# ZihaoW123/UniMM

Hardware: AMD Instinct MI355X
Metric: dialog-sequences/sec (fwd+bwd) at bs=240 seq=256 regions=36(+1 <IMG>) (higher is better)
Workload: dtype bf16; 1 GPU; UniMM-UL sparse training step (BASELINE configs[1]): bert_base_6layer_6conect, sequences_per_image=6, num_negative_samples=5, mask_prob=0.15, dropout on, MLM+UL / NSP / region-KL losses, fwd+bwd, optimizer step not included; global_batch=240, per_gpu_batch=240, seq_len=256, regions=37, parallelism=dp1, executor=eager launches, step_api=loss = combine(losses); loss.backward() (autograd, as train.py:164-168, :315)

## Files before the change

### unimm_amd/csrc/attention.hip

```cpp
#include <type_traits>
#include "common.h"

namespace {

struct AttnParams {
  const bf16_t* q; const bf16_t* k; const bf16_t* v;
  bf16_t* o; float* lse;
  const uint32_t* mask;
  const int* q_off; const int* q_len; const int* k_off; const int* k_len;
  const int* ks_off; const int* ks_len; int ks_ins;
  const int* order;
  int B, H, Tq, Tk, ldq, ldk, ldv, ldo;
  int mask_q_stride, mask_b_stride;
  int parts;
  float scale;
  DropoutArg drop;
};

constexpr float LOG2E = 1.4426950408889634f;
constexpr float LN2 = 0.6931471805599453f;

template <int D> __device__ __forceinline__ int swz(int row) {
  if constexpr (D == 64) { const int t = row >> 1; return (t & 7) ^ ((t & 1) << 2); }
  else return ((row & 3) << 2) | ((row >> 2) & 3);
}

template <int D>
__device__ __forceinline__ void stage_head(const bf16_t* __restrict__ g, int ld, int nrows, int nrows_pad,
                                           char* img, int tid, int nthreads) {
  constexpr int CPR = D / 8;
  constexpr int RPI = 64 / CPR;
  const int wave = tid >> 6, lane = tid & 63, nwaves = nthreads >> 6;
  const int rl = lane / CPR, pc = lane % CPR;
  for (int grp = wave; grp < nrows_pad / RPI; grp += nwaves) {
    const int row = grp * RPI + rl;
    if (row < nrows) {
      const bf16_t* src = g + (size_t)row * ld + ((pc ^ swz<D>(row)) << 3);
      __builtin_amdgcn_global_load_lds(GLB_PTR(src), LDS_PTR(img + grp * 1024), 16, 0, 0);
    } else {
      *reinterpret_cast<u32x4*>(img + grp * 1024 + lane * 16) = u32x4{0u, 0u, 0u, 0u};
    }
  }
}
template <int D>
__device__ __forceinline__ void stage_head_seg(const bf16_t* __restrict__ base, int ld, size_t kbase, size_t sbase, int ins, int slen,
                                               int nrows, int nrows_pad, char* img, int tid, int nthreads) {
  constexpr int CPR = D / 8, RPI = 64 / CPR;
  const int wave = tid >> 6, lane = tid & 63, nwaves = nthreads >> 6;
  const int rl = lane / CPR, pc = lane % CPR;
  for (int grp = wave; grp < nrows_pad / RPI; grp += nwaves) {
    const int row = grp * RPI + rl;
    if (row < nrows) {
      const size_t grow = row < ins ? kbase + row : (row < ins + slen ? sbase + (row - ins) : kbase + (row - slen));
      const bf16_t* src = base + grow * ld + ((pc ^ swz<D>(row)) << 3);
      __builtin_amdgcn_global_load_lds(GLB_PTR(src), LDS_PTR(img + grp * 1024), 16, 0, 0);
    } else {
      *reinterpret_cast<u32x4*>(img + grp * 1024 + lane * 16) = u32x4{0u, 0u, 0u, 0u};
    }
  }
}
__device__ __forceinline__ void stage_wait() { asm volatile("s_waitcnt vmcnt(0)" ::: "memory"); }

template <int D> __device__ __forceinline__ bf16x8 read_row_frag(const char* img, int row, int chunk) {
  return *reinterpret_cast<const bf16x8*>(img + row * (2 * D) + ((chunk ^ swz<D>(row)) << 4));
}

template <int D>
__device__ __forceinline__ bf16x8 read_tr_frag(const char* img, int rowbase, int col0, int lane) {
  const int h = lane >> 5, i = lane & 15, qq = i >> 2, pp = i & 3;
  const int col = col0 + 16 * ((lane >> 4) & 1) + 4 * pp;
  typedef __attribute__((ext_vector_type(8))) short s16x8;
  s16x4 part[2];
#pragma unroll
  for (int jj = 0; jj < 2; ++jj) {
    const int row = rowbase + 8 * jj + 4 * h + qq;
    const int pch = (col >> 3) ^ swz<D>(row);
    part[jj] = __builtin_amdgcn_ds_read_tr16_b64_v4i16(
        (__attribute__((address_space(3))) s16x4*)LDS_PTR(img + row * (2 * D) + pch * 16 + (col & 7) * 2));
  }
  s16x8 v = {part[0][0], part[0][1], part[0][2], part[0][3], part[1][0], part[1][1], part[1][2], part[1][3]};
  return __builtin_bit_cast(bf16x8, v);
}

__device__ __forceinline__ bf16x8 pack8(const float* p) {
  typedef __attribute__((ext_vector_type(4))) unsigned int u4;
  u4 w = {pack2bf(p[0], p[1]), pack2bf(p[2], p[3]), pack2bf(p[4], p[5]), pack2bf(p[6], p[7])};
  return __builtin_bit_cast(bf16x8, w);
}

__device__ __forceinline__ int key_of_reg(int reg, int h) { return (reg & 3) + 8 * (reg >> 2) + 4 * h; }

template <int D>
__device__ __forceinline__ void store_acc_row(bf16_t* __restrict__ g, const f32x16 (&a)[D / 32], float s, int h, bool ok) {
#pragma unroll
  for (int dt = 0; dt < D / 32; ++dt)
#pragma unroll
    for (int qp = 0; qp < 2; ++qp) {
      const uint32_t a0 = pack2bf(a[dt][8 * qp] * s, a[dt][8 * qp + 1] * s), a1 = pack2bf(a[dt][8 * qp + 2] * s, a[dt][8 * qp + 3] * s);
      const uint32_t b0 = pack2bf(a[dt][8 * qp + 4] * s, a[dt][8 * qp + 5] * s), b1 = pack2bf(a[dt][8 * qp + 6] * s, a[dt][8 * qp + 7] * s);
      const auto w0 = __builtin_amdgcn_permlane32_swap(a0, b0, false, false);
      const auto w1 = __builtin_amdgcn_permlane32_swap(a1, b1, false, false);
      if (ok) *reinterpret_cast<u32x4*>(g + 32 * dt + 16 * qp + 8 * h) = u32x4{w0[0], w1[0], w0[1], w1[1]};
    }
}

template <int D, int NKT>
__global__ __launch_bounds__(512, 2) void attn_fwd_kernel(AttnParams p) {
  drop_resolve(p.drop);
  extern __shared__ __attribute__((aligned(16))) char smem[];
  constexpr int KPAD = NKT * 32;
  char* kimg = smem;
  char* vimg = smem + KPAD * 2 * D;
  const int tid = threadIdx.x, wave = tid >> 6, lane = tid & 63;
  const int item = blockIdx.x / p.parts, part = blockIdx.x % p.parts;
  const int b = p.order != nullptr ? p.order[item / p.H] : item / p.H, head = item % p.H;
  const int nwv = blockDim.x >> 6;
  const int r = lane & 31, h = lane >> 5;

  const int Ts_b = p.ks_len ? p.ks_len[b] : 0;
  int Tk_b = (p.k_len ? p.k_len[b] : p.Tk) + Ts_b;
  Tk_b = Tk_b < KPAD ? Tk_b : KPAD;
  const int Tq_b = p.q_len ? p.q_len[b] : p.Tq;
  if (part * (int)(blockDim.x >> 6) * 32 >= Tq_b) return;
  const size_t qbase = p.q_off ? (size_t)p.q_off[b] : (size_t)b * p.Tq;
  const size_t kbase = p.k_off ? (size_t)p.k_off[b] : (size_t)b * p.Tk;
  const size_t sbase = p.ks_off ? (size_t)p.ks_off[b] : 0;
  const int kpad_b = ((Tk_b + 31) & ~31) < KPAD ? ((Tk_b + 31) & ~31) : KPAD;
  stage_head_seg<D>(p.k + head * D, p.ldk, kbase, sbase, p.ks_ins, Ts_b, Tk_b, kpad_b, kimg, tid, blockDim.x);
  stage_head_seg<D>(p.v + head * D, p.ldv, kbase, sbase, p.ks_ins, Ts_b, Tk_b, kpad_b, vimg, tid, blockDim.x);

  int wt = part * nwv + wave;
  int q0, qrow;
  bool qvalid;
  bf16x8 qf[D / 16];
  uint32_t mw[NKT];
#define UNIMM_LOAD_QTILE()                                                                                    \
  {                                                                                                          \
    q0 = wt * 32;                                                                                            \
    qrow = q0 + r;                                                                                           \
    qvalid = qrow < Tq_b;                                                                                    \
    if (!qvalid) qrow = Tq_b - 1;                                                                            \
    const bf16_t* qg_ = p.q + (qbase + qrow) * p.ldq + head * D;                                             \
    _Pragma("unroll") for (int ks = 0; ks < D / 16; ++ks) qf[ks] = *reinterpret_cast<const bf16x8*>(qg_ + 16 * ks + 8 * h); \
    const uint32_t* mp_ = p.mask + (size_t)b * p.mask_b_stride + (size_t)qrow * p.mask_q_stride;            \
    _Pragma("unroll") for (int t = 0; t < NKT; ++t) mw[t] = 32 * t < p.Tk ? mp_[t] : 0u;    \
  }
  UNIMM_LOAD_QTILE()
  stage_wait();
  __syncthreads();
  constexpr bool WALK = D == 64;
  for (bool first = true; wt * 32 < Tq_b && (WALK || first); first = false, wt += nwv * p.parts) {
    if (WALK && !first) UNIMM_LOAD_QTILE()

  f32x16 s[NKT];
#pragma unroll
  for (int t = 0; t < NKT; ++t) {
    f32x16 acc = {};
    if (32 * t < Tk_b) {
#pragma unroll
      for (int ks = 0; ks < D / 16; ++ks) {
        const bf16x8 kf = read_row_frag<D>(kimg, 32 * t + r, 2 * ks + h);
        acc = __builtin_amdgcn_mfma_f32_32x32x16_bf16(kf, qf[ks], acc, 0, 0, 0);
      }
    }
    s[t] = acc;
  }

  const float c1 = p.scale * LOG2E;
  constexpr float MOFF = -10000.0f * LOG2E;
  int tk_here = Tk_b;
  asm volatile("" : "+v"(tk_here));
  float mx = -INFINITY;
#pragma unroll
  for (int t = 0; t < NKT; ++t) {
    if (32 * t >= Tk_b) continue;
    const uint32_t wn = ~(mw[t] >> (4 * h));
    auto scores = [&](auto partial) {
#pragma unroll
      for (int e = 0; e < 16; e += 2) {
        const int kk = (e & 3) + 8 * (e >> 2);
        f32x2v madd;
#pragma unroll
        for (int u = 0; u < 2; ++u) {
          const uint32_t mb = (uint32_t)__builtin_amdgcn_sbfe((int)wn, kk + u, 1) & __builtin_bit_cast(uint32_t, MOFF);
          madd[u] = __uint_as_float(mb);
          if constexpr (decltype(partial)::value)
// ... 26 lines not shown
  if (p.drop.thr != 0u) {
    const uint32_t wl = drop_lin(p.drop, drop_wbase(((uint32_t)b * p.H + head) * p.Tq + (uint32_t)qrow, (uint32_t)p.Tk, 0u) + 2u * (uint32_t)h);
#pragma unroll
    for (int t = 0; t < NKT; ++t) {
      if (32 * t >= Tk_b) continue;
#pragma unroll
      for (int e = 0; e < 16; e += 2) {
        const uint32_t w = drop_fin(p.drop, wl + (uint32_t)((32 * t + key_of_reg(e, 0)) >> 1) * DROP_M1);
        s[t][e] = drop_keep(p.drop, w, 0u) ? s[t][e] : 0.0f;
        s[t][e + 1] = drop_keep(p.drop, w, 1u) ? s[t][e + 1] : 0.0f;
      }
    }
  }

  f32x16 o[D / 32];
#pragma unroll
  for (int dt = 0; dt < D / 32; ++dt) o[dt] = f32x16{};
#pragma unroll
  for (int t = 0; t < NKT; ++t) {
    if (32 * t >= Tk_b) continue;
#pragma unroll
    for (int ss = 0; ss < 2; ++ss) {
      float pv[8];
#pragma unroll
      for (int j = 0; j < 8; ++j) pv[j] = s[t][8 * ss + j];
      const bf16x8 pf = pack8(pv);
#pragma unroll
      for (int dt = 0; dt < D / 32; ++dt) {
        const bf16x8 vf = read_tr_frag<D>(vimg, 32 * t + 16 * ss, 32 * dt, lane);
        o[dt] = __builtin_amdgcn_mfma_f32_32x32x16_bf16(vf, pf, o[dt], 0, 0, 0);
      }
    }
  }

  store_acc_row<D>(p.o + (qbase + (qvalid ? qrow : 0)) * p.ldo + head * D, o, inv, h, qvalid);
  if (qvalid) {
    if (p.lse != nullptr && h == 0) p.lse[((size_t)b * p.H + head) * p.Tq + qrow] = (mx + __log2f(sum)) * LN2;
  }
  }
#undef UNIMM_LOAD_QTILE
}


struct AttnBwdParams {
  const bf16_t* q; const bf16_t* k; const bf16_t* v; const bf16_t* o; const bf16_t* dout;
  const float* lse; float* delta;
  bf16_t* dq; bf16_t* dk; bf16_t* dv;
  const uint32_t* mask;
  const int* q_off; const int* q_len; const int* k_off; const int* k_len;
  const int* order;
  int B, H, Tq, Tk, ldq, ldk, ldv, ldo, lddo, lddq, lddk, lddv;
  int mask_q_stride, mask_b_stride;
  int parts;
  float scale;
  DropoutArg drop;
};

template <int D, int NKT>
__global__ __launch_bounds__(512, 2) void attn_bwd_dq_kernel(AttnBwdParams p) {
  drop_resolve(p.drop);
  extern __shared__ __attribute__((aligned(16))) char smem[];
  constexpr int KPAD = NKT * 32;
  char* kimg = smem;
  char* vimg = smem + KPAD * 2 * D;
  const int tid = threadIdx.x, wave = tid >> 6, lane = tid & 63;
  const int item = blockIdx.x / p.parts, part = blockIdx.x % p.parts;
// ... 266 lines not shown

template <int D>
__device__ __forceinline__ void bwd_stage_row_stats(const AttnBwdParams& p, int b, int head, size_t qbase, int Tq_b, int Tk_b, int qpad_b,
                                                    float* lse_s, float* del_s, uint32_t* mw_s, int mstride, int tid, int nthreads) {
  constexpr int LPR = D / 8;
  for (int i = tid; i < qpad_b; i += nthreads) {
    const size_t stat = ((size_t)b * p.H + head) * p.Tq + i;
    lse_s[i] = i < Tq_b ? -p.lse[stat] * LOG2E : -INFINITY;
  }
  for (int i = tid; i < qpad_b * LPR; i += nthreads) {
    const int row = i / LPR, c = i % LPR;
    float part = 0.f;
    if (row < Tq_b) {
      const u32x4 a = *reinterpret_cast<const u32x4*>(p.dout + (qbase + row) * p.lddo + head * D + 8 * c);
      const u32x4 o = *reinterpret_cast<const u32x4*>(p.o + (qbase + row) * p.ldo + head * D + 8 * c);
#pragma unroll
      for (int e = 0; e < 4; ++e) {
        part = fmaf(__uint_as_float(a[e] << 16), __uint_as_float(o[e] << 16), part);
        part = fmaf(__uint_as_float(a[e] & 0xffff0000u), __uint_as_float(o[e] & 0xffff0000u), part);
      }
    }
#pragma unroll
    for (int o = 1; o < LPR; o <<= 1) part += __shfl_xor(part, o, 64);
    if (c == 0) del_s[row] = part;
  }
  const int nkt_b = (Tk_b + 31) >> 5;
  const uint32_t* mb = p.mask + (size_t)b * p.mask_b_stride;
  for (int i = tid; i < nkt_b * qpad_b; i += nthreads) {
    const int kt = i / qpad_b, qi = i - kt * qpad_b;
    const int qc = qi < Tq_b ? qi : Tq_b - 1;
    mw_s[kt * mstride + qi] = ~mb[(size_t)qc * p.mask_q_stride + kt] | pad_key_bits(Tk_b, kt);
  }
}

struct BwdScoreCtx {
  uint32_t dlane, hbase, halfm, thr16;
  float dsc, c1;
  bool dropping;
};
__device__ __forceinline__ void bwd_score_tile(const AttnBwdParams& p, const BwdScoreCtx& c, const f32x16& sacc, const f32x16& dpacc,
                                               const float* lse_s, const float* del_s, const uint32_t* mrow, int q0, int r, int h,
                                               float (&pd)[16], float (&ds)[16]) {
  constexpr float MOFF = -10000.0f * LOG2E;
  const uint32_t hbase = c.hbase, halfm = c.halfm, dlane = c.dlane, thr16 = c.thr16;
  const float dsc = c.dsc, c1 = c.c1;
  const bool dropping = c.dropping;
#pragma unroll
  for (int g4 = 0; g4 < 4; ++g4) {
    const int qb = q0 + 8 * g4 + 4 * h;
    const f32x4 l4 = *reinterpret_cast<const f32x4*>(lse_s + qb);
    const f32x4 d4 = *reinterpret_cast<const f32x4*>(del_s + qb);
    const u32x4 w4 = *reinterpret_cast<const u32x4*>(mrow + qb);
    uint32_t dwv[4] = {0u, 0u, 0u, 0u};
    const uint32_t odd = (uint32_t)r & 1u;
    if (dropping) {
      const uint32_t ua = (hbase + (uint32_t)(q0 + 8 * g4)) * halfm;
      const uint32_t wa = drop_fin(p.drop, dlane + ua);
      const uint32_t wb = drop_fin(p.drop, dlane + ua + 2u * halfm);
      const uint32_t oa = (uint32_t)__builtin_amdgcn_mov_dpp((int)wa, 0xB1, 0xF, 0xF, true);
      const uint32_t ob = (uint32_t)__builtin_amdgcn_mov_dpp((int)wb, 0xB1, 0xF, 0xF, true);
      dwv[0] = odd ? oa : wa; dwv[1] = odd ? wa : oa; dwv[2] = odd ? ob : wb; dwv[3] = odd ? wb : ob;
    }
    const uint32_t fsh = odd << 4;
#pragma unroll
    for (int i = 0; i < 4; i += 2) {
      const int e = 4 * g4 + i;
// ... 61 lines not shown
  char* pt = qimg + QPAD * 2 * D;
  float* mx_w = reinterpret_cast<float*>(pt + NW * 2 * 2048);
  float* sm_w = mx_w + NW * QPAD;
  const int tid = threadIdx.x, wave = tid >> 6, lane = tid & 63;
  const int item = blockIdx.x;
  const int b = p.order != nullptr ? p.order[item / p.H] : item / p.H, head = item % p.H;
  const int r = lane & 31, h = lane >> 5;
  int Tk_b = p.k_len ? p.k_len[b] : p.Tk;
  Tk_b = Tk_b < KPAD ? Tk_b : KPAD;
  int Tq_b = p.q_len ? p.q_len[b] : p.Tq;
  Tq_b = Tq_b < QPAD ? Tq_b : QPAD;
  const size_t qbase = p.q_off ? (size_t)p.q_off[b] : (size_t)b * p.Tq;
  const size_t kbase = p.k_off ? (size_t)p.k_off[b] : (size_t)b * p.Tk;
  const int kpad_b = (Tk_b + 31) & ~31, qpad_b = (Tq_b + 31) & ~31;
  const int nqt = qpad_b >> 5;
  stage_head<D>(p.v + kbase * p.ldv + head * D, p.ldv, Tk_b, kpad_b, vimg, tid, blockDim.x);
  stage_head<D>(p.q + qbase * p.ldq + head * D, p.ldq, Tq_b, qpad_b, qimg, tid, blockDim.x);

  const int wt = wave;
  const bool wave_on = wt * 32 < Tk_b;
  int krow = wt * 32 + r;
  if (krow >= Tk_b) krow = Tk_b - 1;
  const bf16_t* kg = p.k + (kbase + krow) * p.ldk + head * D;
  bf16x8 kf[D / 16];
#pragma unroll
  for (int ks = 0; ks < D / 16; ++ks) kf[ks] = *reinterpret_cast<const bf16x8*>(kg + 16 * ks + 8 * h);
  uint32_t mw[2];
  int qrow[2];
#pragma unroll
  for (int qt = 0; qt < 2; ++qt) {
    int q = 32 * qt + r;
    q = q < Tq_b ? q : Tq_b - 1;
    qrow[qt] = q;
    mw[qt] = 32 * wt < p.Tk ? p.mask[(size_t)b * p.mask_b_stride + (size_t)q * p.mask_q_stride + wt] : 0u;
  }
  stage_wait();
  __syncthreads();

  const float c1 = p.scale * LOG2E;
  constexpr float MOFF = -10000.0f * LOG2E;
  f32x16 s[2];
#pragma unroll
  for (int qt = 0; qt < 2; ++qt) {
    float mxl = -INFINITY;
    s[qt] = f32x16{};
    if (wave_on && qt < nqt) {
      f32x16 acc = {};
#pragma unroll
      for (int ks = 0; ks < D / 16; ++ks) {
        const bf16x8 qf = read_row_frag<D>(qimg, 32 * qt + r, 2 * ks + h);
        acc = __builtin_amdgcn_mfma_f32_32x32x16_bf16(kf[ks], qf, acc, 0, 0, 0);
      }
      const uint32_t wn = ~(mw[qt] >> (4 * h));
      const bool partial = 32 * (wt + 1) > Tk_b;
#pragma unroll
      for (int e = 0; e < 16; e += 2) {
        const int kk = (e & 3) + 8 * (e >> 2);
        f32x2v madd;
#pragma unroll
        for (int u = 0; u < 2; ++u) {
          const uint32_t mb = (uint32_t)__builtin_amdgcn_sbfe((int)wn, kk + u, 1) & __builtin_bit_cast(uint32_t, MOFF);
          madd[u] = __uint_as_float(mb);
          if (partial) madd[u] = (32 * wt + kk + u + 4 * h) < Tk_b ? madd[u] : -INFINITY;
        }
        const f32x2v v = f32x2v{acc[e], acc[e + 1]} * c1 + madd;
        acc[e] = v.x; acc[e + 1] = v.y;
        mxl = fmaxf(mxl, fmaxf(v.x, v.y));
// ... 65 lines not shown
    const float inv = (p.drop.thr != 0u ? p.drop.scale : 1.0f) / sum;
    const int q = 32 * qt2 + r;
    const bool qvalid = q < Tq_b;
    store_acc_row<32>(p.o + (qbase + (qvalid ? q : 0)) * p.ldo + head * D + 32 * dt, o1, inv, h, qvalid);
    if (dt == 0 && qvalid && h == 0 && p.lse != nullptr) p.lse[((size_t)b * p.H + head) * p.Tq + q] = (mx + __log2f(sum)) * LN2;
  }
}

template <int NQT>
__global__ __launch_bounds__(512, 2) void attn_bwd_fused_kernel(AttnBwdParams p) {
  constexpr int D = 64;
  drop_resolve(p.drop);
  extern __shared__ __attribute__((aligned(16))) char smem[];
  constexpr int QPAD = NQT * 32;
  constexpr int AS = D + 4;
  char* qimg = smem;
  char* doimg = smem + QPAD * 2 * D;
  float* lse_s = reinterpret_cast<float*>(smem + 2 * QPAD * 2 * D);
  float* del_s = lse_s + QPAD;
  uint32_t* mw_s = reinterpret_cast<uint32_t*>(del_s + QPAD);
  char* scr = reinterpret_cast<char*>(mw_s + 8 * QPAD);
  float* acc = reinterpret_cast<float*>(scr + 8 * 2048);
  int* turn = reinterpret_cast<int*>(acc + QPAD * AS);
  const int tid = threadIdx.x, wave = tid >> 6, lane = tid & 63;
  const int item = blockIdx.x;
  const int b = p.order != nullptr ? p.order[item / p.H] : item / p.H, head = item % p.H;
  const int wt = wave;
  const int r = lane & 31, h = lane >> 5;

  const int Tq_b = p.q_len ? p.q_len[b] : p.Tq, Tk_b = p.k_len ? p.k_len[b] : p.Tk;
  const size_t qbase = p.q_off ? (size_t)p.q_off[b] : (size_t)b * p.Tq;
  const size_t kbase = p.k_off ? (size_t)p.k_off[b] : (size_t)b * p.Tk;
  const int qpad_b = ((Tq_b + 31) & ~31) < QPAD ? ((Tq_b + 31) & ~31) : QPAD;
  stage_head<D>(p.q + qbase * p.ldq + head * D, p.ldq, Tq_b, qpad_b, qimg, tid, blockDim.x);
  stage_head<D>(p.dout + qbase * p.lddo + head * D, p.lddo, Tq_b, qpad_b, doimg, tid, blockDim.x);
  bwd_stage_row_stats<D>(p, b, head, qbase, Tq_b, Tk_b, qpad_b, lse_s, del_s, mw_s, QPAD, tid, blockDim.x);
  if (tid < NQT) turn[tid] = 0;

  int krow = wt * 32 + r;
  const bool kvalid = krow < Tk_b;
  const bool wave_on = wt * 32 < Tk_b;
  if (!kvalid) krow = Tk_b - 1;
  const size_t grow = kbase + krow;
  const bf16_t* kg = p.k + grow * p.ldk + head * D;
  const bf16_t* vg = p.v + grow * p.ldv + head * D;
  bf16x8 kf[D / 16], vf[D / 16];
#pragma unroll
  for (int ks = 0; ks < D / 16; ++ks) {
    kf[ks] = *reinterpret_cast<const bf16x8*>(kg + 16 * ks + 8 * h);
    vf[ks] = *reinterpret_cast<const bf16x8*>(vg + 16 * ks + 8 * h);
  }
  bf16x8 ktf[2][2];
  {
    char* kt = reinterpret_cast<char*>(acc) + wave * (32 * 2 * D);
#pragma unroll
    for (int ks = 0; ks < D / 16; ++ks) {
      const u32x4 v = kvalid ? __builtin_bit_cast(u32x4, kf[ks]) : u32x4{0u, 0u, 0u, 0u};
      *reinterpret_cast<u32x4*>(kt + r * (2 * D) + (((2 * ks + h) ^ swz<D>(r)) << 4)) = v;
    }
#pragma unroll
    for (int ss = 0; ss < 2; ++ss) {
      ktf[0][ss] = read_tr_frag<D>(kt, 16 * ss, 0, lane);
      ktf[1][ss] = read_tr_frag<D>(kt, 16 * ss, 32, lane);
    }
  }
  stage_wait();
  __syncthreads();

  f32x16 dk[D / 32], dv[D / 32];
#pragma unroll
  for (int dt = 0; dt < D / 32; ++dt) { dk[dt] = f32x16{}; dv[dt] = f32x16{}; }
  const uint32_t* mrow = mw_s + wt * QPAD;
  char* ws = scr + wave * 2048;
  const uint32_t hbase = ((uint32_t)b * p.H + head) * (uint32_t)p.Tq;
  const uint32_t halfw = ((uint32_t)p.Tk + 1u) >> 1, halfm = halfw * DROP_M1;
  const uint32_t dlane = drop_lin(p.drop, (4u * (uint32_t)h + ((uint32_t)r & 1u)) * halfw + ((uint32_t)(wt * 32 + r) >> 1));
  const float c1 = p.scale * LOG2E;
  const bool dropping = p.drop.thr != 0u;
  const uint32_t thr16 = dropping ? (p.drop.thr >> 16) : 0u;
  const float dsc = dropping ? p.drop.scale : 1.0f;
  const BwdScoreCtx sctx{dlane, hbase, halfm, thr16, dsc, c1, dropping};

  if (wave_on) {
#pragma unroll 1
  for (int qt = 0; qt < NQT; ++qt) {
    if (32 * qt >= Tq_b) break;
    f32x16 sacc = {}, dpacc = {};
#pragma unroll
    for (int ks = 0; ks < D / 16; ++ks) {
      const bf16x8 qf = read_row_frag<D>(qimg, 32 * qt + r, 2 * ks + h);
      sacc = __builtin_amdgcn_mfma_f32_32x32x16_bf16(qf, kf[ks], sacc, 0, 0, 0);
      const bf16x8 df = read_row_frag<D>(doimg, 32 * qt + r, 2 * ks + h);
      dpacc = __builtin_amdgcn_mfma_f32_32x32x16_bf16(df, vf[ks], dpacc, 0, 0, 0);
    }
    float pd[16], ds[16];
    bwd_score_tile(p, sctx, sacc, dpacc, lse_s, del_s, mrow, 32 * qt, r, h, pd, ds);
#pragma unroll
    for (int g4 = 0; g4 < 4; ++g4)
// ... 51 lines not shown
    if (q >= Tq_b) continue;
    float v[8];
#pragma unroll
    for (int j = 0; j < 8; ++j) v[j] = acc[q * AS + 8 * c + j] * p.scale;
    *reinterpret_cast<u32x4*>(p.dq + (qbase + q) * p.lddq + head * D + 8 * c) =
        u32x4{pack2bf(v[0], v[1]), pack2bf(v[2], v[3]), pack2bf(v[4], v[5]), pack2bf(v[6], v[7])};
  }
}

template <int NQT>
__global__ __launch_bounds__(512, 2) void attn_bwd_fewq128_kernel(AttnBwdParams p) {
  constexpr int D = 128;
  static_assert(NQT == 2, "the (sequence, head) item's queries are two 32-row tiles: P / dS of both stay in registers for phase 2");
  drop_resolve(p.drop);
  extern __shared__ __attribute__((aligned(16))) char smem[];
  constexpr int QPAD = NQT * 32;
  char* qimg = smem;
  char* doimg = smem + QPAD * 2 * D;
  float* lse_s = reinterpret_cast<float*>(smem + 2 * QPAD * 2 * D);
  float* del_s = lse_s + QPAD;
  uint32_t* mw_s = reinterpret_cast<uint32_t*>(del_s + QPAD);
  char* scr = reinterpret_cast<char*>(mw_s + 8 * QPAD);
  char* kimgs = scr + 8 * NQT * 2048;
  const int tid = threadIdx.x, wave = tid >> 6, lane = tid & 63;
  const int item = blockIdx.x;
  const int b = p.order != nullptr ? p.order[item / p.H] : item / p.H, head = item % p.H;
  const int wt = wave;
  const int r = lane & 31, h = lane >> 5;

  const int Tq_b = p.q_len ? p.q_len[b] : p.Tq, Tk_b = p.k_len ? p.k_len[b] : p.Tk;
  const size_t qbase = p.q_off ? (size_t)p.q_off[b] : (size_t)b * p.Tq;
  const size_t kbase = p.k_off ? (size_t)p.k_off[b] : (size_t)b * p.Tk;
  const int qpad_b = ((Tq_b + 31) & ~31) < QPAD ? ((Tq_b + 31) & ~31) : QPAD;
  stage_head<D>(p.q + qbase * p.ldq + head * D, p.ldq, Tq_b, qpad_b, qimg, tid, blockDim.x);
  stage_head<D>(p.dout + qbase * p.lddo + head * D, p.lddo, Tq_b, qpad_b, doimg, tid, blockDim.x);
  bwd_stage_row_stats<D>(p, b, head, qbase, Tq_b, Tk_b, qpad_b, lse_s, del_s, mw_s, QPAD, tid, blockDim.x);

  int krow = wt * 32 + r;
  const bool kvalid = krow < Tk_b;
  const bool wave_on = wt * 32 < Tk_b;
  if (!kvalid) krow = Tk_b - 1;
  const size_t grow = kbase + krow;
  const bf16_t* kg = p.k + grow * p.ldk + head * D;
  const bf16_t* vg = p.v + grow * p.ldv + head * D;
  bf16x8 kf[D / 16], vf[D / 16];
#pragma unroll
  for (int ks = 0; ks < D / 16; ++ks) {
    kf[ks] = *reinterpret_cast<const bf16x8*>(kg + 16 * ks + 8 * h);
    vf[ks] = *reinterpret_cast<const bf16x8*>(vg + 16 * ks + 8 * h);
  }
  char* kimg = kimgs + wave * (32 * 2 * D);
#pragma unroll
  for (int ks = 0; ks < D / 16; ++ks) {
    const u32x4 v = kvalid ? __builtin_bit_cast(u32x4, kf[ks]) : u32x4{0u, 0u, 0u, 0u};
    *reinterpret_cast<u32x4*>(kimg + r * (2 * D) + (((2 * ks + h) ^ swz<D>(r)) << 4)) = v;
  }
  stage_wait();
  __syncthreads();

  bf16x8 pfr[NQT][2], dsfr[NQT][2];
#pragma unroll
  for (int qt = 0; qt < NQT; ++qt)
#pragma unroll
    for (int ss = 0; ss < 2; ++ss) { pfr[qt][ss] = bf16x8{}; dsfr[qt][ss] = bf16x8{}; }
  const uint32_t* mrow = mw_s + wt * QPAD;
  const uint32_t hbase = ((uint32_t)b * p.H + head) * (uint32_t)p.Tq;
  const uint32_t halfw = ((uint32_t)p.Tk + 1u) >> 1, halfm = halfw * DROP_M1;
  const uint32_t dlane = drop_lin(p.drop, (4u * (uint32_t)h + ((uint32_t)r & 1u)) * halfw + ((uint32_t)(wt * 32 + r) >> 1));
  const float c1 = p.scale * LOG2E;
  const bool dropping = p.drop.thr != 0u;
  const uint32_t thr16 = dropping ? (p.drop.thr >> 16) : 0u;
  const float dsc = dropping ? p.drop.scale : 1.0f;
  const BwdScoreCtx sctx{dlane, hbase, halfm, thr16, dsc, c1, dropping};

  if (wave_on) {
#pragma unroll
  for (int qt = 0; qt < NQT; ++qt) {
    if (32 * qt < Tq_b) {
    f32x16 sacc = {}, dpacc = {};
#pragma unroll
    for (int ks = 0; ks < D / 16; ++ks) {
      const bf16x8 qf = read_row_frag<D>(qimg, 32 * qt + r, 2 * ks + h);
      sacc = __builtin_amdgcn_mfma_f32_32x32x16_bf16(qf, kf[ks], sacc, 0, 0, 0);
      const bf16x8 df = read_row_frag<D>(doimg, 32 * qt + r, 2 * ks + h);
      dpacc = __builtin_amdgcn_mfma_f32_32x32x16_bf16(df, vf[ks], dpacc, 0, 0, 0);
    }
    float pd[16], ds[16];
    bwd_score_tile(p, sctx, sacc, dpacc, lse_s, del_s, mrow, 32 * qt, r, h, pd, ds);
    char* ws = scr + (wave * NQT + qt) * 2048;
// ... 46 lines not shown
            dqa[0] = __builtin_amdgcn_mfma_f32_32x32x16_bf16(ktf, dstf, dqa[0], 0, 0, 0);
          }
        }
      }
      const int q = 32 * qt + r;
      const bool ok = q < Tq_b;
      store_acc_row<32>(p.dq + (qbase + (ok ? q : 0)) * p.lddq + head * D + 32 * dt, dqa, p.scale, h, ok);
    }
  }
}

__global__ __launch_bounds__(512, 2) void attn_bwd_fewk128_kernel(AttnBwdParams p) {
  constexpr int D = 128, NKT = 2, KPAD = NKT * 32, QMAX = 256, NQT = QMAX / 32;
  drop_resolve(p.drop);
  extern __shared__ __attribute__((aligned(16))) char smem[];
  char* kimg = smem;
  char* vimg = smem + KPAD * 2 * D;
  float* lse_s = reinterpret_cast<float*>(smem + 2 * KPAD * 2 * D);
  float* del_s = lse_s + QMAX;
  uint32_t* mw_s = reinterpret_cast<uint32_t*>(del_s + QMAX);
  char* scr = reinterpret_cast<char*>(mw_s + NKT * QMAX);
  char* bfrag = scr + 8 * 6144;
  const int tid = threadIdx.x, wave = tid >> 6, lane = tid & 63;
  const int item = blockIdx.x;
  const int b = p.order != nullptr ? p.order[item / p.H] : item / p.H, head = item % p.H;
  const int wq = wave;
  const int r = lane & 31, h = lane >> 5;

  const int Tq_b = p.q_len ? p.q_len[b] : p.Tq, Tk_b = p.k_len ? p.k_len[b] : p.Tk;
  const size_t qbase = p.q_off ? (size_t)p.q_off[b] : (size_t)b * p.Tq;
  const size_t kbase = p.k_off ? (size_t)p.k_off[b] : (size_t)b * p.Tk;
  const int qpad_b = ((Tq_b + 31) & ~31) < QMAX ? ((Tq_b + 31) & ~31) : QMAX;
  const int kpad_b = ((Tk_b + 31) & ~31) < KPAD ? ((Tk_b + 31) & ~31) : KPAD;
  stage_head<D>(p.k + kbase * p.ldk + head * D, p.ldk, Tk_b, kpad_b, kimg, tid, blockDim.x);
  stage_head<D>(p.v + kbase * p.ldv + head * D, p.ldv, Tk_b, kpad_b, vimg, tid, blockDim.x);
  bwd_stage_row_stats<D>(p, b, head, qbase, Tq_b, Tk_b, qpad_b, lse_s, del_s, mw_s, QMAX, tid, blockDim.x);

  int qrow = wq * 32 + r;
  const bool qvalid = qrow < Tq_b;
  const bool wave_on = wq * 32 < Tq_b;
  if (!qvalid) qrow = Tq_b - 1;
  const size_t grow = qbase + qrow;
  const bf16_t* qg = p.q + grow * p.ldq + head * D;
  const bf16_t* dg = p.dout + grow * p.lddo + head * D;
  bf16x8 qf[D / 16], dof[D / 16];
#pragma unroll
  for (int ks = 0; ks < D / 16; ++ks) {
    qf[ks] = *reinterpret_cast<const bf16x8*>(qg + 16 * ks + 8 * h);
    dof[ks] = *reinterpret_cast<const bf16x8*>(dg + 16 * ks + 8 * h);
  }
  stage_wait();
  __syncthreads();

  char* wsb = scr + wave * 6144;
  const uint32_t hbase = ((uint32_t)b * p.H + head) * (uint32_t)p.Tq;
  const uint32_t halfw = ((uint32_t)p.Tk + 1u) >> 1, halfm = halfw * DROP_M1;
  const float c1 = p.scale * LOG2E;
  const bool dropping = p.drop.thr != 0u;
  const uint32_t thr16 = dropping ? (p.drop.thr >> 16) : 0u;
  const float dsc = dropping ? p.drop.scale : 1.0f;

  if (wave_on) {
#pragma unroll
  for (int kt = 0; kt < NKT; ++kt) {
    if (32 * kt < Tk_b) {
    const uint32_t* mrow = mw_s + kt * QMAX;
    char* ws = wsb + kt * 2048;
    const uint32_t dlane = drop_lin(p.drop, (4u * (uint32_t)h + ((uint32_t)r & 1u)) * halfw + ((uint32_t)(kt * 32 + r) >> 1));
    const BwdScoreCtx sctx{dlane, hbase, halfm, thr16, dsc, c1, dropping};
    f32x16 sacc = {}, dpacc = {};
#pragma unroll
    for (int ks = 0; ks < D / 16; ++ks) {
      const bf16x8 kfr = read_row_frag<D>(kimg, 32 * kt + r, 2 * ks + h);
      sacc = __builtin_amdgcn_mfma_f32_32x32x16_bf16(qf[ks], kfr, sacc, 0, 0, 0);
      const bf16x8 vfr = read_row_frag<D>(vimg, 32 * kt + r, 2 * ks + h);
      dpacc = __builtin_amdgcn_mfma_f32_32x32x16_bf16(dof[ks], vfr, dpacc, 0, 0, 0);
    }
    float pd[16], ds[16];
    bwd_score_tile(p, sctx, sacc, dpacc, lse_s, del_s, mrow, 32 * wq, r, h, pd, ds);
#pragma unroll
    for (int g4 = 0; g4 < 4; ++g4)
      *reinterpret_cast<u32x2*>(ws + r * 64 + (((2 * g4 + h) ^ tile64_swz(r)) << 3)) =
          u32x2{pack2bf(ds[4 * g4], ds[4 * g4 + 1]), pack2bf(ds[4 * g4 + 2], ds[4 * g4 + 3])};
// ... 924 lines not shown
```

Measured before the change: 6089 dialog-sequences/sec.

## Slim attention forward score path to raise occupancy for D64 short-key tiles

Rewrites the forward attention softmax section to hold scores as packed float pairs. Mask handling is split into specialised fully-unmasked, masked and partial-tile variants, selected by a wave ballot. Scheduling barriers interleave MFMA with LDS reads, and V fragments are prefetched in groups. Launch bounds for D=64, NKT=2 rise from 2 to 3 blocks per CU, trading register budget for occupancy. It also skips the mask load in the backward kernel for inactive waves.

After: 6112 dialog-sequences/sec (median of 3 runs). Within noise of the previous version (+0.4%).

```diff
diff --git a/unimm_amd/csrc/attention.hip b/unimm_amd/csrc/attention.hip
--- a/unimm_amd/csrc/attention.hip
+++ b/unimm_amd/csrc/attention.hip
@@ -16,6 +16,10 @@
   float scale;
   DropoutArg drop;
 };
+
+#ifndef UNIMM_ATTN_SCORE_DIET
+#define UNIMM_ATTN_SCORE_DIET 1
+#endif
 
 constexpr float LOG2E = 1.4426950408889634f;
 constexpr float LN2 = 0.6931471805599453f;
@@ -105,7 +109,7 @@
 }
 
 template <int D, int NKT>
-__global__ __launch_bounds__(512, 2) void attn_fwd_kernel(AttnParams p) {
+__global__ __launch_bounds__(512, UNIMM_ATTN_SCORE_DIET && D == 64 && NKT == 2 ? 3 : 2) void attn_fwd_kernel(AttnParams p) {
   drop_resolve(p.drop);
   extern __shared__ __attribute__((aligned(16))) char smem[];
   constexpr int KPAD = NKT * 32;
@@ -149,9 +153,121 @@
   stage_wait();
   __syncthreads();
   constexpr bool WALK = D == 64;
+#if UNIMM_ATTN_SCORE_DIET
+  int bfe_one = 1;
+  asm volatile("" : "+s"(bfe_one));
+#endif
   for (bool first = true; wt * 32 < Tq_b && (WALK || first); first = false, wt += nwv * p.parts) {
     if (WALK && !first) UNIMM_LOAD_QTILE()
 
+#if UNIMM_ATTN_SCORE_DIET
+  const float c1 = p.scale * LOG2E;
+  constexpr float MOFF = -10000.0f * LOG2E;
+  int tk_here = Tk_b;
+  asm volatile("" : "+v"(tk_here));
+  f32x2v sp[NKT][8];
+  float mx = -INFINITY;
+#pragma unroll
+  for (int t = 0; t < NKT; ++t) {
+    if (32 * t >= Tk_b) continue;
+    f32x16 acc = {};
+#pragma unroll
+    for (int ks = 0; ks < D / 16; ++ks) {
+      const bf16x8 kf = read_row_frag<D>(kimg, 32 * t + r, 2 * ks + h);
+      acc = __builtin_amdgcn_mfma_f32_32x32x16_bf16(kf, qf[ks], acc, 0, 0, 0);
+    }
+    if constexpr (D == 64) {
+      __builtin_amdgcn_sched_group_barrier(0x100, D / 16, 0);
+      __builtin_amdgcn_sched_group_barrier(0x008, D / 16, 0);
+    }
+    const uint32_t wn = ~(mw[t] >> (4 * h));
+    auto scores = [&](auto masked, auto partial) {
+#pragma unroll
+      for (int j = 0; j < 8; ++j) {
+        const int kk = key_of_reg(2 * j, 0);
+        f32x2v madd = {0.0f, 0.0f};
+#pragma unroll
+        for (int u = 0; u < 2; ++u) {
+          if constexpr (decltype(masked)::value)
+            madd[u] = __uint_as_float((uint32_t)__builtin_amdgcn_sbfe((int)wn, kk + u, bfe_one) & __builtin_bit_cast(uint32_t, MOFF));
+          if constexpr (decltype(partial)::value)
+            madd[u] = (32 * t + kk + u + 4 * h) < tk_here ? madd[u] : -INFINITY;
+        }
+        const f32x2v v = f32x2v{acc[2 * j], acc[2 * j + 1]} * c1 + madd;
+        sp[t][j] = v;
+        mx = fmaxf(mx, fmaxf(v.x, v.y));
+      }
+    };
+    if (32 * (t + 1) > Tk_b) scores(std::true_type{}, std::true_type{});
+    else if (__builtin_amdgcn_ballot_w64((wn & 0x0f0f0f0fu) != 0u) != 0ull) scores(std::true_type{}, std::false_type{});
+    else scores(std::false_type{}, std::false_type{});
+  }
+  mx = fmaxf(mx, __shfl_xor(mx, 32, 64));
+  f32x2v sum2 = {0.f, 0.f};
+#pragma unroll
+  for (int t = 0; t < NKT; ++t) {
+    if (32 * t >= Tk_b) continue;
+#pragma unroll
+    for (int j = 0; j < 8; ++j) {
+      const f32x2v a = sp[t][j] - mx;
+      const float p0 = __builtin_amdgcn_exp2f(a.x), p1 = __builtin_amdgcn_exp2f(a.y);
+      sp[t][j] = f32x2v{p0, p1};
+      sum2 += f32x2v{p0, p1};
+    }
+  }
+  float sum = sum2.x + sum2.y;
+  sum += __shfl_xor(sum, 32, 64);
+  const float inv = (p.drop.thr != 0u ? p.drop.scale : 1.0f) / sum;
+
+  if (p.drop.thr != 0u) {
+    uint32_t wl = drop_lin(p.drop, drop_wbase(((uint32_t)b * p.H + head) * p.Tq + (uint32_t)qrow, (uint32_t)p.Tk, 0u) + 2u * (uint32_t)h);
+    asm volatile("" : "+v"(wl));
+#pragma unroll
+    for (int t = 0; t < NKT; ++t) {
+      if (32 * t >= Tk_b) continue;
+#pragma unroll
+      for (int j = 0; j < 8; ++j) {
+        uint32_t w = wl + (uint32_t)((32 * t + key_of_reg(2 * j, 0)) >> 1) * DROP_M1;
+        w = __builtin_amdgcn_bitop3_b32(w, w >> 15, p.drop.key2, 0x96) * DROP_M2;
+        w ^= w >> 16;
+        sp[t][j].x = drop_keep(p.drop, w, 0u) ? sp[t][j].x : 0.0f;
+        sp[t][j].y = drop_keep(p.drop, w, 1u) ? sp[t][j].y : 0.0f;
+      }
+    }
+  }
+
+  f32x16 o[D / 32];
+#pragma unroll
+  for (int dt = 0; dt < D / 32; ++dt) o[dt] = f32x16{};
+  constexpr int SSG = D == 64 ? 2 : 1;
+#pragma unroll
+  for (int t = 0; t < NKT; ++t) {
+    if (32 * t >= Tk_b) continue;
+#pragma unroll
+    for (int s0 = 0; s0 < 2; s0 += SSG) {
+      bf16x8 vf[SSG][D / 32];
+#pragma unroll
+      for (int ss = 0; ss < SSG; ++ss)
+#pragma unroll
+        for (int dt = 0; dt < D / 32; ++dt) vf[ss][dt] = read_tr_frag<D>(vimg, 32 * t + 16 * (s0 + ss), 32 * dt, lane);
+#pragma unroll
+      for (int ss = 0; ss < SSG; ++ss) {
+        float pv[8];
+#pragma unroll
+        for (int j = 0; j < 4; ++j) { pv[2 * j] = sp[t][4 * (s0 + ss) + j].x; pv[2 * j + 1] = sp[t][4 * (s0 + ss) + j].y; }
+        const bf16x8 pf = pack8(pv);
+#pragma unroll
+        for (int dt = 0; dt < D / 32; ++dt) o[dt] = __builtin_amdgcn_mfma_f32_32x32x16_bf16(vf[ss][dt], pf, o[dt], 0, 0, 0);
+      }
+      __builtin_amdgcn_sched_group_barrier(0x100, 2 * SSG * (D / 32), 0);
+#pragma unroll
+      for (int ss = 0; ss < SSG; ++ss) {
+        __builtin_amdgcn_sched_group_barrier(0x002, 4, 0);
+        __builtin_amdgcn_sched_group_barrier(0x008, D / 32, 0);
+      }
+    }
+  }
+#else
   f32x16 s[NKT];
 #pragma unroll
   for (int t = 0; t < NKT; ++t) {
@@ -244,6 +360,8 @@
       }
     }
   }
+
+#endif
 
   store_acc_row<D>(p.o + (qbase + (qvalid ? qrow : 0)) * p.ldo + head * D, o, inv, h, qvalid);
   if (qvalid) {
@@ -703,7 +821,7 @@
     int q = 32 * qt + r;
     q = q < Tq_b ? q : Tq_b - 1;
     qrow[qt] = q;
-    mw[qt] = 32 * wt < p.Tk ? p.mask[(size_t)b * p.mask_b_stride + (size_t)q * p.mask_q_stride + wt] : 0u;
+    mw[qt] = wave_on && 32 * wt < p.Tk ? p.mask[(size_t)b * p.mask_b_stride + (size_t)q * p.mask_q_stride + wt] : 0u;
   }
   stage_wait();
   __syncthreads();
```

## Overlap attention-backward row-stat loads with K/V and Q/dO staging

Applied to the files above, without the earlier changes.

The backward attention kernels' prologue is restructured so the global loads for the row statistics (lse, dO·O delta inputs, mask words) are all issued into registers first. Asynchronous LDS staging is split into an issue phase and a separate zero-fill phase, and the delta/mask reductions are consumed after the per-wave K/V or Q/dO register loads. This is meant to hide prologue memory latency, which was serialized in the old bwd_stage_row_stats loop. In exchange it uses more registers per thread (which could lower occupancy) and assumes a fixed 512-thread block and QPAD<=512.

After: 5958 dialog-sequences/sec before, 5991 dialog-sequences/sec after, median of 4. About the same (+0.6%).

```diff
diff --git a/unimm_amd/csrc/attention.hip b/unimm_amd/csrc/attention.hip
--- a/unimm_amd/csrc/attention.hip
+++ b/unimm_amd/csrc/attention.hip
@@ -60,6 +60,28 @@
   }
 }
 __device__ __forceinline__ void stage_wait() { asm volatile("s_waitcnt vmcnt(0)" ::: "memory"); }
+template <int D>
+__device__ __forceinline__ void stage_head_issue(const bf16_t* __restrict__ g, int ld, int nrows, int nrows_pad, char* img, int tid,
+                                                 int nthreads) {
+  constexpr int CPR = D / 8, RPI = 64 / CPR;
+  const int wave = tid >> 6, lane = tid & 63, nwaves = nthreads >> 6;
+  const int rl = lane / CPR, pc = lane % CPR;
+  for (int grp = wave; grp < nrows_pad / RPI; grp += nwaves) {
+    const int row = grp * RPI + rl;
+    if (row < nrows) {
+      const bf16_t* src = g + (size_t)row * ld + ((pc ^ swz<D>(row)) << 3);
+      __builtin_amdgcn_global_load_lds(GLB_PTR(src), LDS_PTR(img + grp * 1024), 16, 0, 0);
+    }
+  }
+}
+template <int D>
+__device__ __forceinline__ void stage_head_zero(int nrows, int nrows_pad, char* img, int tid, int nthreads) {
+  constexpr int CPR = D / 8, RPI = 64 / CPR;
+  const int wave = tid >> 6, lane = tid & 63, nwaves = nthreads >> 6;
+  const int rl = lane / CPR;
+  for (int grp = wave; grp < nrows_pad / RPI; grp += nwaves)
+    if (grp * RPI + rl >= nrows) *reinterpret_cast<u32x4*>(img + grp * 1024 + lane * 16) = u32x4{0u, 0u, 0u, 0u};
+}
 
 template <int D> __device__ __forceinline__ bf16x8 read_row_frag(const char* img, int row, int chunk) {
   return *reinterpret_cast<const bf16x8*>(img + row * (2 * D) + ((chunk ^ swz<D>(row)) << 4));
@@ -576,6 +598,78 @@
     mw_s[kt * mstride + qi] = ~mb[(size_t)qc * p.mask_q_stride + kt] | pad_key_bits(Tk_b, kt);
   }
 }
+
+#ifndef UNIMM_ATTN_BWD_STAGE
+#define UNIMM_ATTN_BWD_STAGE 1
+#endif
+template <int D, int QPAD, int NKT>
+struct BwdRowStats {
+  static constexpr int LPR = D / 8, NT = 512;
+  static constexpr int DS = QPAD * LPR / NT, MS = (NKT * QPAD + NT - 1) / NT;
+  static_assert(QPAD <= NT && DS * NT == QPAD * LPR, "one lse slot per thread; whole delta slots");
+  float lse;
+  u32x4 a[DS], o[DS];
+  uint32_t mw[MS];
+
+  __device__ __forceinline__ void issue(const AttnBwdParams& p, int b, int head, size_t qbase, int Tq_b, int Tk_b, int qpad_b, int tid) {
+    lse = 0.f;
+#pragma unroll
+    for (int s = 0; s < DS; ++s) { a[s] = u32x4{0u, 0u, 0u, 0u}; o[s] = u32x4{0u, 0u, 0u, 0u}; }
+#pragma unroll
+    for (int s = 0; s < MS; ++s) mw[s] = 0u;
+    if (Tq_b <= 0) return;
+    const int last = Tq_b - 1;
+    lse = p.lse[((size_t)b * p.H + head) * p.Tq + (tid < Tq_b ? tid : last)];
+#pragma unroll
+    for (int s = 0; s < DS; ++s) {
+      const int i = tid + s * NT;
+      const int row = i / LPR, c = i % LPR;
+      const size_t grow = qbase + (row < Tq_b ? row : last);
+      a[s] = *reinterpret_cast<const u32x4*>(p.dout + grow * p.lddo + head * D + 8 * c);
+      o[s] = *reinterpret_cast<const u32x4*>(p.o + grow * p.ldo + head * D + 8 * c);
+    }
+    const int ktlast = Tk_b > 0 ? (Tk_b - 1) >> 5 : 0;
+    const uint32_t* mb = p.mask + (size_t)b * p.mask_b_stride;
+#pragma unroll
+    for (int s = 0; s < MS; ++s) {
+      const int i = tid + s * NT;
+      const int kt = i / qpad_b, qi = i - kt * qpad_b;
+      const int qc = qi < Tq_b ? qi : last;
+      mw[s] = mb[(size_t)qc * p.mask_q_stride + (kt < ktlast ? kt : ktlast)];
+    }
+    __builtin_amdgcn_sched_barrier(0);
+  }
+
+  __device__ __forceinline__ void consume(float* lse_s, float* del_s, uint32_t* mw_s, int mstride, int Tq_b, int Tk_b, int qpad_b,
+                                          int tid) const {
+    if (tid < qpad_b) lse_s[tid] = tid < Tq_b ? -lse * LOG2E : -INFINITY;
+#pragma unroll
+    for (int s = 0; s < DS; ++s) {
+      const int i = tid + s * NT;
+      const int row = i / LPR, c = i % LPR;
+      float part = 0.f;
+      if (row < Tq_b) {
+#pragma unroll
+        for (int e = 0; e < 4; ++e) {
+          part = fmaf(__uint_as_float(a[s][e] << 16), __uint_as_float(o[s][e] << 16), part);
+          part = fmaf(__uint_as_float(a[s][e] & 0xffff0000u), __uint_as_float(o[s][e] & 0xffff0000u), part);
+        }
+      }
+#pragma unroll
+      for (int x = 1; x < LPR; x <<= 1) part += __shfl_xor(part, x, 64);
+      if (i < qpad_b * LPR && c == 0) del_s[row] = part;
+    }
+    const int nkt_b = (Tk_b + 31) >> 5;
+#pragma unroll
+    for (int s = 0; s < MS; ++s) {
+      const int i = tid + s * NT;
+      if (i < nkt_b * qpad_b) {
+        const int kt = i / qpad_b, qi = i - kt * qpad_b;
+        mw_s[kt * mstride + qi] = ~mw[s] | pad_key_bits(Tk_b, kt);
+      }
+    }
+  }
+};
 
 struct BwdScoreCtx {
   uint32_t dlane, hbase, halfm, thr16;
@@ -835,10 +929,15 @@
   const size_t qbase = p.q_off ? (size_t)p.q_off[b] : (size_t)b * p.Tq;
   const size_t kbase = p.k_off ? (size_t)p.k_off[b] : (size_t)b * p.Tk;
   const int qpad_b = ((Tq_b + 31) & ~31) < QPAD ? ((Tq_b + 31) & ~31) : QPAD;
+#if UNIMM_ATTN_BWD_STAGE
+  stage_head_issue<D>(p.q + qbase * p.ldq + head * D, p.ldq, Tq_b, qpad_b, qimg, tid, blockDim.x);
+  stage_head_issue<D>(p.dout + qbase * p.lddo + head * D, p.lddo, Tq_b, qpad_b, doimg, tid, blockDim.x);
+#else
   stage_head<D>(p.q + qbase * p.ldq + head * D, p.ldq, Tq_b, qpad_b, qimg, tid, blockDim.x);
   stage_head<D>(p.dout + qbase * p.lddo + head * D, p.lddo, Tq_b, qpad_b, doimg, tid, blockDim.x);
   bwd_stage_row_stats<D>(p, b, head, qbase, Tq_b, Tk_b, qpad_b, lse_s, del_s, mw_s, QPAD, tid, blockDim.x);
   if (tid < NQT) turn[tid] = 0;
+#endif
 
   int krow = wt * 32 + r;
   const bool kvalid = krow < Tk_b;
@@ -853,6 +952,13 @@
     kf[ks] = *reinterpret_cast<const bf16x8*>(kg + 16 * ks + 8 * h);
     vf[ks] = *reinterpret_cast<const bf16x8*>(vg + 16 * ks + 8 * h);
   }
+#if UNIMM_ATTN_BWD_STAGE
+  BwdRowStats<D, QPAD, 8> stats;
+  stats.issue(p, b, head, qbase, Tq_b, Tk_b, qpad_b, tid);
+  stage_head_zero<D>(Tq_b, qpad_b, qimg, tid, blockDim.x);
+  stage_head_zero<D>(Tq_b, qpad_b, doimg, tid, blockDim.x);
+  if (tid < NQT) turn[tid] = 0;
+#endif
   bf16x8 ktf[2][2];
   {
     char* kt = reinterpret_cast<char*>(acc) + wave * (32 * 2 * D);
@@ -867,6 +973,9 @@
       ktf[1][ss] = read_tr_frag<D>(kt, 16 * ss, 32, lane);
     }
   }
+#if UNIMM_ATTN_BWD_STAGE
+  stats.consume(lse_s, del_s, mw_s, QPAD, Tq_b, Tk_b, qpad_b, tid);
+#endif
   stage_wait();
   __syncthreads();
 
@@ -984,9 +1093,14 @@
   const size_t qbase = p.q_off ? (size_t)p.q_off[b] : (size_t)b * p.Tq;
   const size_t kbase = p.k_off ? (size_t)p.k_off[b] : (size_t)b * p.Tk;
   const int qpad_b = ((Tq_b + 31) & ~31) < QPAD ? ((Tq_b + 31) & ~31) : QPAD;
+#if UNIMM_ATTN_BWD_STAGE
+  stage_head_issue<D>(p.q + qbase * p.ldq + head * D, p.ldq, Tq_b, qpad_b, qimg, tid, blockDim.x);
+  stage_head_issue<D>(p.dout + qbase * p.lddo + head * D, p.lddo, Tq_b, qpad_b, doimg, tid, blockDim.x);
+#else
   stage_head<D>(p.q + qbase * p.ldq + head * D, p.ldq, Tq_b, qpad_b, qimg, tid, blockDim.x);
   stage_head<D>(p.dout + qbase * p.lddo + head * D, p.lddo, Tq_b, qpad_b, doimg, tid, blockDim.x);
   bwd_stage_row_stats<D>(p, b, head, qbase, Tq_b, Tk_b, qpad_b, lse_s, del_s, mw_s, QPAD, tid, blockDim.x);
+#endif
 
   int krow = wt * 32 + r;
   const bool kvalid = krow < Tk_b;
@@ -1001,12 +1115,21 @@
     kf[ks] = *reinterpret_cast<const bf16x8*>(kg + 16 * ks + 8 * h);
     vf[ks] = *reinterpret_cast<const bf16x8*>(vg + 16 * ks + 8 * h);
   }
+#if UNIMM_ATTN_BWD_STAGE
+  BwdRowStats<D, QPAD, 8> stats;
+  stats.issue(p, b, head, qbase, Tq_b, Tk_b, qpad_b, tid);
+  stage_head_zero<D>(Tq_b, qpad_b, qimg, tid, blockDim.x);
+  stage_head_zero<D>(Tq_b, qpad_b, doimg, tid, blockDim.x);
+#endif
   char* kimg = kimgs + wave * (32 * 2 * D);
 #pragma unroll
   for (int ks = 0; ks < D / 16; ++ks) {
     const u32x4 v = kvalid ? __builtin_bit_cast(u32x4, kf[ks]) : u32x4{0u, 0u, 0u, 0u};
     *reinterpret_cast<u32x4*>(kimg + r * (2 * D) + (((2 * ks + h) ^ swz<D>(r)) << 4)) = v;
   }
+#if UNIMM_ATTN_BWD_STAGE
+  stats.consume(lse_s, del_s, mw_s, QPAD, Tq_b, Tk_b, qpad_b, tid);
+#endif
   stage_wait();
   __syncthreads();
 
@@ -1119,9 +1242,14 @@
   const size_t kbase = p.k_off ? (size_t)p.k_off[b] : (size_t)b * p.Tk;
   const int qpad_b = ((Tq_b + 31) & ~31) < QMAX ? ((Tq_b + 31) & ~31) : QMAX;
   const int kpad_b = ((Tk_b + 31) & ~31) < KPAD ? ((Tk_b + 31) & ~31) : KPAD;
+#if UNIMM_ATTN_BWD_STAGE
+  stage_head_issue<D>(p.k + kbase * p.ldk + head * D, p.ldk, Tk_b, kpad_b, kimg, tid, blockDim.x);
+  stage_head_issue<D>(p.v + kbase * p.ldv + head * D, p.ldv, Tk_b, kpad_b, vimg, tid, blockDim.x);
+#else
   stage_head<D>(p.k + kbase * p.ldk + head * D, p.ldk, Tk_b, kpad_b, kimg, tid, blockDim.x);
   stage_head<D>(p.v + kbase * p.ldv + head * D, p.ldv, Tk_b, kpad_b, vimg, tid, blockDim.x);
   bwd_stage_row_stats<D>(p, b, head, qbase, Tq_b, Tk_b, qpad_b, lse_s, del_s, mw_s, QMAX, tid, blockDim.x);
+#endif
 
   int qrow = wq * 32 + r;
   const bool qvalid = qrow < Tq_b;
@@ -1136,6 +1264,13 @@
     qf[ks] = *reinterpret_cast<const bf16x8*>(qg + 16 * ks + 8 * h);
     dof[ks] = *reinterpret_cast<const bf16x8*>(dg + 16 * ks + 8 * h);
   }
+#if UNIMM_ATTN_BWD_STAGE
+  BwdRowStats<D, QMAX, NKT> stats;
+  stats.issue(p, b, head, qbase, Tq_b, Tk_b, qpad_b, tid);
+  stage_head_zero<D>(Tk_b, kpad_b, kimg, tid, blockDim.x);
+  stage_head_zero<D>(Tk_b, kpad_b, vimg, tid, blockDim.x);
+  stats.consume(lse_s, del_s, mw_s, QMAX, Tq_b, Tk_b, qpad_b, tid);
+#endif
   stage_wait();
   __syncthreads();
 
```
